# ratschlab/projects2014-metagenome

Hardware: AMD Instinct MI355X
Metric: k-mers/s ingested into BOSS (k=31, 150 bp reads) (higher is better)
Workload: dtype u64

## Files before the change

projects2014-metagenome_amd/csrc/boss_pipeline.hip:

```cpp
#include <hip/hip_runtime.h>

#include <algorithm>
#include <cmath>
#include <atomic>
#include <chrono>
#include <cstdio>
#include <cstring>
#include <mutex>
#include <stdexcept>
#include <string>
#include <type_traits>
#include <vector>

#include <sys/types.h>
#include <unistd.h>

#include "../../include/mtg_boss.h"
#include "boss_kernels.hpp"
#include "comm.hpp"
#include "dbg_io.hpp"
#include "dbg_device.hpp"
#include "dist_kernels.hpp"
#include "superkmer.hpp"
#include "extract_partition.hpp"
// ... 658 lines not shown
template <int L>
static MsdPlan msd_plan(const Ctx &c, uint64_t n, unsigned nbits, double dup) {
    const double LIMIT = (double)LocalTraits<L>::LIMIT / 2;
    const unsigned dmax = MSD_DBITS;
    unsigned T = 0;
    while (T < nbits && T < 3 * dmax && (double)n / dup / (double)(1ull << T) > LIMIT / kPlanDiv)
        ++T;
    MsdPlan p{};
    p.levels = (T + dmax - 1) / dmax;
    if (c.min_levels > p.levels && T >= c.min_levels) p.levels = c.min_levels;
    for (unsigned l = 1; l <= p.levels; ++l) p.digit_end[l] = T * l / p.levels;
    return p;
}

static void note_bucket_index(Ctx &c, const void *keys, uint64_t n, const uint64_t *start, unsigned shift);

template <int L>
static MsdPlan rc_plan(const Ctx &c, uint64_t n, unsigned nbits) {
    return msd_plan<L>(c, L == 2 && c.rc_wide ? std::max<uint64_t>(1, n / 2) : n, nbits, 1.0);
}

template <int L>
struct RcMerge {
    const Key<L> *ck;
    const uint32_t *cv;
    uint64_t nc;
    Key<L> *out;
    uint32_t *outc;
    bool done = false;
    uint64_t *istart = nullptr;
    unsigned ib = 0;
};

__global__ void spec_caps_kernel(const uint32_t *__restrict__ sample, uint64_t nb, uint32_t stride,
                                 uint32_t *__restrict__ cap, bool tiny, uint64_t blo, uint64_t bhi,
                                 uint32_t align = 0) {
    const uint64_t b = (uint64_t)blockIdx.x * blockDim.x + threadIdx.x;
    if (b >= nb) return;
    if (b < blo || b >= bhi) {
        cap[b] = 0;
        return;
    }
    uint32_t v = tiny ? (uint32_t)(((uint64_t)sample[b] * stride) / 2)
                      : (uint32_t)(((uint64_t)sample[b] * stride * 6) / 5) + 512u;
    if (align) v = (v + align - 1) / align * align;
    cap[b] = v;
}

__global__ void spec_tile_fill_kernel(const uint64_t *__restrict__ bstart, const unsigned long long *__restrict__ cur,
                                      uint64_t nb, uint32_t tile, uint32_t *__restrict__ tv) {
    const uint64_t b = (uint64_t)blockIdx.x * blockDim.x + threadIdx.x;
    if (b >= nb) return;
    const uint64_t s = bstart[b], e = bstart[b + 1], k = cur[b];
    for (uint64_t t = s / tile; t < e / tile; ++t) {
        const uint64_t t0 = t * tile;
        tv[t] = (uint32_t)(k <= t0 ? 0 : min<uint64_t>(tile, k - t0));
    }
}

__global__ void spec_counts_kernel(const uint64_t *__restrict__ bstart, const unsigned long long *__restrict__ cur,
                                   uint64_t nb, uint32_t *__restrict__ cnt) {
    const uint64_t b = (uint64_t)blockIdx.x * blockDim.x + threadIdx.x;
    if (b < nb) cnt[b] = (uint32_t)(cur[b] - bstart[b]);
}

template <typename F>
static void bucket_pieces(uint64_t lo, uint64_t hi, F &&launch) {
    constexpr uint64_t CH = 1ull << 22;
    for (uint64_t g0 = lo; g0 < hi; g0 += CH) launch(g0, (unsigned)std::min(CH, hi - g0));
}

static void ensure_compact(Ctx &c) {
    if (!c.gap.valid) return;
    c.gap.valid = false;
    if (!c.gap.nb) return;
    bucket_pieces(0, c.gap.nb, [&](uint64_t g0, unsigned cnt) {
        group_gather_kernel<1, false><<<dim3(cnt), dim3(256), 0, c.stream>>>(
            (const Key<1> *)c.gap.keys, nullptr, c.gap.bstart, c.gap.ustart, (Key<1> *)c.gap.dst, nullptr, nullptr, 0,
            nullptr, nullptr, g0);
        HIP_CHECK(hipGetLastError());
    });
}

template <int L, bool COUNTED>
static uint64_t spec_final_level(Ctx &c, Key<L> **keys, uint32_t **vals, uint64_t n, unsigned nbits, unsigned bp,
                                 unsigned bb, uint32_t cmax, bool distinct, RcMerge<L> *rm,
                                 const Ctx::GroupIndex &cidx, bool fine = false, Key<L> *spare = nullptr) {
    if constexpr (L != 1) {
        return ~0ull;
    } else {
        constexpr double KB = COUNTED ? 12.0 : 8.0;
        if (distinct != (rm != nullptr)) return ~0ull;
        if (rm && !c.spec_rc) return ~0ull;
        if (rm && !(cidx.keys == (const void *)rm->ck && cidx.n == rm->nc && cidx.bits == bb && cidx.nbits == nbits &&
                    bb <= 32 && (!rm->istart || rm->ib >= bb)))
            return ~0ull;
        constexpr uint32_t SS = 8;
        constexpr int TILE = MsdTraits<L>::TILE;
        const bool g1 = bp && c.gap1_n && !rm;
        const uint64_t npos = g1 ? c.gap1_n : n;
        const uint32_t *tv = g1 ? c.gap1_tv : nullptr;
        const uint64_t tiles = ceil_div(npos, TILE);
        if (c.use_lsd || !c.spec_final || tiles < 64 * SS || bb - bp > 9 || bb > 24) return ~0ull;
        if (g1) fine = true;
        const uint64_t nb = 1ull << bb;
        const bool gap_out = !COUNTED && c.defer_gather_req && c.defer_gather && c.want_gidx;
        const bool inplace = !rm && c.spec_inplace && !gap_out;
        if (COUNTED) spare = nullptr;
        if (!spare) {
            const uint64_t fr = c.ws.free_bytes();
            if ((double)n * KB * 1.4 * (inplace ? 1.0 : 2.0) > 0.5 * (double)fr + (double)c.ws.held_slot(Workspace::SPEC_A) +
                                                  (double)c.ws.held_slot(Workspace::SPEC_B) +
                                                  (double)c.ws.held_slot(Workspace::SPEC_AC) +
                                                  (double)c.ws.held_slot(Workspace::SPEC_BC))
                return ~0ull;
        }
        uint32_t *h = (uint32_t *)c.ws.get(Workspace::MSD_COUNTS, nb * 4);
        HIP_CHECK(hipMemsetAsync(h, 0, nb * 4, c.stream));
        constexpr uint32_t GT = 8;
        msd_hist_kernel<L><<<dim3((unsigned)(fine ? ceil_div(tiles, GT) : ceil_div(tiles, SS))), dim3(MSD_BLOCK), 0,
                             c.stream>>>(*keys, npos, nbits, bb, bp, h, fine ? 1 : SS, fine ? SS : 1, fine ? GT : 1, tv);
        HIP_CHECK(hipGetLastError());
        uint64_t blo = 0, bhi = nb;
        if (g1 && c.gap1_hi > c.gap1_lo) {
            blo = c.gap1_lo << (bb - bp);
            bhi = std::min<uint64_t>(nb, c.gap1_hi << (bb - bp));
        } else if (bp && !g1) {
            Key<L> ends[2];
            HIP_CHECK(hipMemcpyAsync(&ends[0], *keys, sizeof(Key<L>), hipMemcpyDeviceToHost, c.stream));
            HIP_CHECK(hipMemcpyAsync(&ends[1], *keys + (n - 1), sizeof(Key<L>), hipMemcpyDeviceToHost, c.stream));
            HIP_CHECK(hipStreamSynchronize(c.stream));
            blo = (ends[0].w[0] >> (nbits - bp)) << (bb - bp);
            bhi = std::min<uint64_t>(nb, ((ends[1].w[0] >> (nbits - bp)) + 1) << (bb - bp));
        }
        uint32_t *cap = (uint32_t *)c.ws.get(Workspace::SPEC_CAP, nb * 4);
        spec_caps_kernel<<<dim3((unsigned)ceil_div(nb, 256)), dim3(256), 0, c.stream>>>(h, nb, SS, cap, c.spec_tiny,
                                                                                        blo, bhi);
        HIP_CHECK(hipGetLastError());
        uint64_t *bstart = (uint64_t *)c.ws.get(Workspace::MSD_BSTART, (nb + 1) * 8);
        {
            uint32_t ep;
            const uint64_t st = ceil_div(nb, 4096);
            uint64_t *desc = acquire_desc(c, st, &ep);
            HIP_CHECK(hipMemsetAsync(&c.small->counter, 0, 4, c.stream));
            scan_counts_kernel<<<dim3((unsigned)st), dim3(512), 0, c.stream>>>(cap, nb, bstart, desc, ep,
                                                                              &c.small->counter, &c.small->error);
            HIP_CHECK(hipGetLastError());
        }
        const uint64_t C = read_u64(c, (const unsigned long long *)(bstart + nb));
        if (spare && C * sizeof(Key<L>) > c.spec_into_bytes) spare = nullptr;
        if (!spare) {
            const uint64_t fr = c.ws.free_bytes();
            const double need = (double)C * KB * (rm || inplace ? 1.0 : 2.0);
            const double have = 0.9 * (double)fr + (double)c.ws.held_slot(Workspace::SPEC_A) +
                                (double)c.ws.held_slot(Workspace::SPEC_AC) +
                                (rm ? 0.0 : (double)c.ws.held_slot(Workspace::SPEC_B) +
                                                (double)c.ws.held_slot(Workspace::SPEC_BC));
            if (need > have) {
                if (c.debug) fprintf(stderr, "[mtg debug] speculative level: capacity %lu does not fit, exact level\n",
                                     (unsigned long)C);
                return ~0ull;
            }
        }
        Key<L> *sa = spare ? spare : (Key<L> *)c.ws.get(Workspace::SPEC_A, C * sizeof(Key<L>));
        uint32_t *sac = COUNTED ? (uint32_t *)c.ws.get(Workspace::SPEC_AC, C * 4) : nullptr;
        auto *cur = (unsigned long long *)c.ws.get(Workspace::SPEC_CUR, nb * 8);
        HIP_CHECK(hipMemcpyAsync(cur, bstart, nb * 8, hipMemcpyDeviceToDevice, c.stream));
        HIP_CHECK(hipMemsetAsync(&c.small->spec_ovf, 0, 4, c.stream));
        EventTimer tm(c.stream);
        tm.mark();
        msd_partition_kernel<L, COUNTED><<<dim3((unsigned)xcd_grid(tiles)), dim3(MSD_BLOCK), 0, c.stream>>>(
            *keys, sa, COUNTED ? *vals : nullptr, sac, npos, nbits, bb, bp, cur, 1,
            (const unsigned long long *)(bstart + 1), &c.small->spec_ovf, tv);
        HIP_CHECK(hipGetLastError());
        tm.mark();
        uint32_t povf = 0;
        HIP_CHECK(hipMemcpyAsync(&povf, &c.small->spec_ovf, 4, hipMemcpyDeviceToHost, c.stream));
        HIP_CHECK(hipStreamSynchronize(c.stream));
        if (c.track_partition && c.radix_launches == 0) {
            c.radix_ms += tm.ms(0, 1);
            c.radix_launches += 1;
            c.radix_bytes += 2.0 * n * KB;
        }
        if (povf) {
            if (c.debug) fprintf(stderr, "[mtg debug] speculative level: a bucket overflowed, exact level\n");
            c.radix_ms = 0, c.radix_launches = 0, c.radix_bytes = 0;
            ++c.timings.spec_fallbacks;
            return ~0ull;
        }
        auto consumed_gap1 = [&]() {
            if (g1) c.gap1_n = 0, c.gap1_tv = nullptr, c.gap1_lo = c.gap1_hi = 0;
        };
        if (rm) {
            uint32_t *cnt = (uint32_t *)c.ws.get(Workspace::SPEC_CAP, nb * 4);
            spec_counts_kernel<<<dim3((unsigned)ceil_div(nb, 256)), dim3(256), 0, c.stream>>>(bstart, cur, nb, cnt);
            HIP_CHECK(hipGetLastError());
            uint64_t *gbase = (uint64_t *)c.ws.get(Workspace::MSD_USTART, (nb + 1) * 8);
            {
                uint32_t ep;
                const uint64_t st = ceil_div(nb, 4096);
                uint64_t *desc = acquire_desc(c, st, &ep);
                HIP_CHECK(hipMemsetAsync(&c.small->counter, 0, 4, c.stream));
                scan_counts_kernel<<<dim3((unsigned)st), dim3(512), 0, c.stream>>>(cnt, nb, gbase, desc, ep,
                                                                                  &c.small->counter, &c.small->error);
                HIP_CHECK(hipGetLastError());
            }
            constexpr int CAP = MergeLocalTraits<L>::CAP;
            uint32_t *olist = (uint32_t *)c.ws.get(Workspace::MSD_OVF, nb * 4);
            HIP_CHECK(hipMemsetAsync(&c.small->counter, 0, 4, c.stream));
            uint64_t *istart = rm->istart;
            const bool gapped = c.gap.valid && c.gap.dst == (const void *)rm->ck;
            const Key<L> *ck = gapped ? (const Key<L> *)c.gap.keys : rm->ck;
            const uint64_t *cgap = gapped ? c.gap.bstart : nullptr;
            uint64_t mlo = 0, mhi = nb;
            if (bp && !g1 && !gapped && rm->nc) {
                Key<L> e[4];
                HIP_CHECK(hipMemcpyAsync(&e[0], *keys, sizeof(Key<L>), hipMemcpyDeviceToHost, c.stream));
                HIP_CHECK(hipMemcpyAsync(&e[1], *keys + (n - 1), sizeof(Key<L>), hipMemcpyDeviceToHost, c.stream));
                HIP_CHECK(hipMemcpyAsync(&e[2], rm->ck, sizeof(Key<L>), hipMemcpyDeviceToHost, c.stream));
                HIP_CHECK(hipMemcpyAsync(&e[3], rm->ck + (rm->nc - 1), sizeof(Key<L>), hipMemcpyDeviceToHost, c.stream));
                HIP_CHECK(hipStreamSynchronize(c.stream));
                auto top = [&](const Key<L> &x) { return bits_at(shr(x, nbits - bp), 0, 32); };
                mlo = std::min(top(e[0]), top(e[2])) << (bb - bp);
                mhi = std::min<uint64_t>(nb, (std::max(top(e[1]), top(e[3])) + 1) << (bb - bp));
                if (istart && mlo < mhi) {
                    const uint64_t ilo = mlo << (rm->ib - bb), ihi = mhi << (rm->ib - bb), iend = 1ull << rm->ib;
                    if (ilo) fill_u64_kernel<<<dim3((unsigned)std::min<uint64_t>(ceil_div(ilo, 256), 4096)), dim3(256), 0,
                                               c.stream>>>(istart, 0, ilo, 0);
                    if (ihi < iend)
                        fill_u64_kernel<<<dim3((unsigned)std::min<uint64_t>(ceil_div(iend - ihi, 256), 4096)), dim3(256),
                                          0, c.stream>>>(istart, ihi, iend, n + rm->nc);
                    HIP_CHECK(hipGetLastError());
                } else if (mlo >= mhi) {
                    mlo = 0, mhi = nb;
                }
            }
            bucket_pieces(mlo, mhi, [&](uint64_t g0, unsigned cnt) {
                local_merge_kernel<L, COUNTED, CAP><<<dim3(cnt), dim3(512), 0, c.stream>>>(
                    sa, sac, bstart, nullptr, nullptr, ck, rm->cv, cidx.start, rm->out, rm->outc, olist,
                    &c.small->counter, bb, nbits, rm->ib, istart, cur, gbase, cgap, g0, c.merge_it);
                HIP_CHECK(hipGetLastError());
            });
            uint32_t novf = 0;
            HIP_CHECK(hipMemcpyAsync(&novf, &c.small->counter, 4, hipMemcpyDeviceToHost, c.stream));
            HIP_CHECK(hipStreamSynchronize(c.stream));
            if (novf) {
                const uint32_t nlist = novf;
                HIP_CHECK(hipMemsetAsync(&c.small->counter, 0, 4, c.stream));
                bucket_pieces(0, nlist, [&](uint64_t g0, unsigned cnt) {
                    local_merge_kernel<L, COUNTED, 2 * CAP><<<dim3(cnt), dim3(512), 0, c.stream>>>(
                        sa, sac, bstart, nullptr, olist + g0, ck, rm->cv, cidx.start, rm->out, rm->outc, nullptr,
                        &c.small->counter, bb, nbits, rm->ib, istart, cur, gbase, cgap, 0, c.merge_it);
                    HIP_CHECK(hipGetLastError());
                });
                HIP_CHECK(hipMemcpyAsync(&novf, &c.small->counter, 4, hipMemcpyDeviceToHost, c.stream));
                HIP_CHECK(hipStreamSynchronize(c.stream));
// ... 79 lines not shown
                fprintf(stderr, "[mtg debug] speculative level: n=%lu capacity=%lu (%.2fx) -> %lu distinct, left in buckets\n",
                        (unsigned long)n, (unsigned long)C, (double)C / (double)n, (unsigned long)u);
            return u;
        }
        const bool index = c.want_gidx;
        const bool rindex = !index && c.ridx.start && bb <= c.ridx.bits;
        uint64_t *gi = index ? (uint64_t *)c.ws.get(Workspace::CANON_IDX, (nb + 2) * 8) : rindex ? c.ridx.start : nullptr;
        const unsigned ib = rindex ? c.ridx.bits : bb;
        if (index || rindex) HIP_CHECK(hipMemsetAsync(&c.small->gidx_bad, 0, 4, c.stream));
        if (c.sort_out && (c.sort_out_cap == ~0ull || read_u64(c, (const unsigned long long *)(ustart + nb)) <= c.sort_out_cap)) {
            *keys = (Key<L> *)c.sort_out;
            if (COUNTED) *vals = c.sort_out_vals;
        }
        bucket_pieces(0, nb, [&](uint64_t g0, unsigned cnt) {
            group_gather_kernel<L, COUNTED><<<dim3(cnt), dim3(256), 0, c.stream>>>(
                sb, sbc, bstart, ustart, *keys, COUNTED ? *vals : nullptr, nullptr, nbits - ib, gi, &c.small->gidx_bad,
                g0, ib - bb, rindex ? c.ridx.off : 0, rindex ? c.ridx.lo : 0, rindex ? c.ridx.hi : ~0ull);
            HIP_CHECK(hipGetLastError());
        });
        uint64_t u = 0;
        uint32_t ibad = 0;
        HIP_CHECK(hipMemcpyAsync(&u, ustart + nb, 8, hipMemcpyDeviceToHost, c.stream));
        if (index) {
            HIP_CHECK(hipMemcpyAsync(gi + nb, ustart + nb, 8, hipMemcpyDeviceToDevice, c.stream));
            HIP_CHECK(hipMemcpyAsync(gi + nb + 1, ustart + nb, 8, hipMemcpyDeviceToDevice, c.stream));
        }
        if (index || rindex) HIP_CHECK(hipMemcpyAsync(&ibad, &c.small->gidx_bad, 4, hipMemcpyDeviceToHost, c.stream));
        HIP_CHECK(hipStreamSynchronize(c.stream));
        if (index && !ibad) c.gidx = Ctx::GroupIndex{*keys, u, bb, nbits, gi};
        if (rindex) c.ridx.written = !ibad;
        consumed_gap1();
        ++c.timings.spec_levels;
        if (fine) ++c.timings.spec_fine_levels;
        if (c.debug)
            fprintf(stderr, "[mtg debug] speculative level: n=%lu capacity=%lu (%.2fx) -> %lu distinct\n",
                    (unsigned long)n, (unsigned long)C, (double)C / (double)n, (unsigned long)u);
        return u;
    }
}

template <int L, bool COUNTED>
static bool spec_mid_level(Ctx &c, Key<L> **keys, Key<L> **alt, uint64_t n, unsigned nbits, unsigned bp, unsigned bb) {
    if constexpr (L != 1 || COUNTED) {
        return false;
    } else {
        constexpr int TILE = MsdTraits<L>::TILE;
        constexpr uint32_t SS = 8;
        const uint64_t tiles = ceil_div(n, TILE);
        if (c.use_lsd || !c.spec_final || tiles < 64 * SS || bb - bp > 9 || bb > 24 || !bp) return false;
        const uint64_t nb = 1ull << bb;
        uint32_t *h = (uint32_t *)c.ws.get(Workspace::MSD_COUNTS, nb * 4);
        HIP_CHECK(hipMemsetAsync(h, 0, nb * 4, c.stream));
        msd_hist_kernel<L><<<dim3((unsigned)ceil_div(tiles, SS)), dim3(MSD_BLOCK), 0, c.stream>>>(*keys, n, nbits, bb, bp, h,
                                                                                                SS, 1, 1, nullptr);
        HIP_CHECK(hipGetLastError());
        Key<L> ends[2];
        HIP_CHECK(hipMemcpyAsync(&ends[0], *keys, sizeof(Key<L>), hipMemcpyDeviceToHost, c.stream));
        HIP_CHECK(hipMemcpyAsync(&ends[1], *keys + (n - 1), sizeof(Key<L>), hipMemcpyDeviceToHost, c.stream));
        HIP_CHECK(hipStreamSynchronize(c.stream));
        const uint64_t lo1 = ends[0].w[0] >> (nbits - bp), hi1 = ends[1].w[0] >> (nbits - bp);
        const uint64_t blo = lo1 << (bb - bp), bhi = std::min<uint64_t>(nb, (hi1 + 1) << (bb - bp));
        uint32_t *cap = (uint32_t *)c.ws.get(Workspace::SPEC_CAP, nb * 4);
        spec_caps_kernel<<<dim3((unsigned)ceil_div(nb, 256)), dim3(256), 0, c.stream>>>(h, nb, SS, cap, c.spec_tiny, blo,
                                                                                        bhi, (uint32_t)TILE);
        HIP_CHECK(hipGetLastError());
        uint64_t *bstart = (uint64_t *)c.ws.get(Workspace::MSD_BSTART, (nb + 1) * 8);
        {
            uint32_t ep;
            const uint64_t st = ceil_div(nb, 4096);
            uint64_t *desc = acquire_desc(c, st, &ep);
            HIP_CHECK(hipMemsetAsync(&c.small->counter, 0, 4, c.stream));
            scan_counts_kernel<<<dim3((unsigned)st), dim3(512), 0, c.stream>>>(cap, nb, bstart, desc, ep,
                                                                              &c.small->counter, &c.small->error);
            HIP_CHECK(hipGetLastError());
        }
        const uint64_t C = read_u64(c, (const unsigned long long *)(bstart + nb));
        if (C * sizeof(Key<L>) > c.spec_mid_bytes) {
            if (c.debug) fprintf(stderr, "[mtg debug] speculative middle level: capacity %lu does not fit\n", (unsigned long)C);
            return false;
        }
        auto *cur = (unsigned long long *)c.ws.get(Workspace::SPEC_CUR, nb * 8);
        HIP_CHECK(hipMemcpyAsync(cur, bstart, nb * 8, hipMemcpyDeviceToDevice, c.stream));
        HIP_CHECK(hipMemsetAsync(&c.small->spec_ovf, 0, 4, c.stream));
        msd_partition_kernel<L, false><<<dim3((unsigned)xcd_grid(tiles)), dim3(MSD_BLOCK), 0, c.stream>>>(
            *keys, *alt, nullptr, nullptr, n, nbits, bb, bp, cur, 1, (const unsigned long long *)(bstart + 1),
            &c.small->spec_ovf, nullptr);
        HIP_CHECK(hipGetLastError());
        const uint64_t ntv = C / TILE;
        uint32_t *tv = (uint32_t *)c.ws.get(Workspace::SPEC_MID_TV, std::max<uint64_t>(ntv, 1) * 4);
        spec_tile_fill_kernel<<<dim3((unsigned)ceil_div(nb, 256)), dim3(256), 0, c.stream>>>(bstart, cur, nb, TILE, tv);
        HIP_CHECK(hipGetLastError());
        uint32_t povf = 0;
        HIP_CHECK(hipMemcpyAsync(&povf, &c.small->spec_ovf, 4, hipMemcpyDeviceToHost, c.stream));
        HIP_CHECK(hipStreamSynchronize(c.stream));
        if (povf) {
            if (c.debug) fprintf(stderr, "[mtg debug] speculative middle level: a bucket overflowed, exact level\n");
            ++c.timings.spec_fallbacks;
            return false;
        }
        std::swap(*keys, *alt);
        c.gap1_n = C;
        c.gap1_tv = tv;
        c.gap1_lo = blo, c.gap1_hi = bhi;
        ++c.timings.spec_levels;
        if (c.debug)
            fprintf(stderr, "[mtg debug] speculative middle level: n=%lu capacity=%lu (%.2fx)\n", (unsigned long)n,
                    (unsigned long)C, (double)C / (double)n);
        return true;
    }
}

template <int L, bool COUNTED>
static uint64_t msd_sort_unique(Ctx &c, Key<L> **keys, Key<L> **alt, uint32_t **vals,
                                uint32_t **valt, uint64_t n, unsigned nbits, uint32_t cmax,
                                double dup, const uint32_t *hist1 = nullptr, bool distinct = false,
                                const std::vector<uint64_t> *runs = nullptr, bool level1_done = false,
                                RcMerge<L> *rm = nullptr, const MsdPlan *force_plan = nullptr) {
    const Ctx::GroupIndex saved_gidx = c.gidx;
    c.gidx = Ctx::GroupIndex{};
    if (n == 0) return 0;
    auto lazy_alt = [&]() {
        if (!*alt) *alt = (Key<L> *)c.ws.get(Workspace::KB, n * sizeof(Key<L>));
        if (COUNTED && !*valt) *valt = (uint32_t *)c.ws.get(Workspace::CB, n * 4);
    };
    constexpr uint32_t LIMIT = LocalTraits<L>::LIMIT;
    constexpr int TILE = MsdTraits<L>::TILE;
    const uint64_t tiles = ceil_div(n, TILE);
    const MsdPlan plan = force_plan ? *force_plan : msd_plan<L>(c, n, nbits, dup);
    unsigned levels = plan.levels;
    unsigned digit_end[4] = {plan.digit_end[0], plan.digit_end[1], plan.digit_end[2], plan.digit_end[3]};
    unsigned b = 0;
    uint64_t *bstart = nullptr;
    uint64_t nbuckets = 1;
    auto run_level = [&](unsigned lev) {
        if (digit_end[lev] == 0) digit_end[lev] = std::min(nbits, digit_end[lev - 1] + 8);
        const unsigned bb = digit_end[lev], bp = digit_end[lev - 1];
        nbuckets = 1ull << bb;
        const uint32_t *cnt = hist1;
        const bool g1 = c.gap1_n && (lev == 2 ? level1_done : lev == 3);
        const uint64_t npos = g1 ? c.gap1_n : n, ltiles = g1 ? ceil_div(npos, TILE) : tiles;
        const uint32_t *tv = g1 ? c.gap1_tv : nullptr;
        if (lev != 1 || !hist1) {
            uint32_t *h = (uint32_t *)c.ws.get(Workspace::MSD_COUNTS, nbuckets * 4);
            HIP_CHECK(hipMemsetAsync(h, 0, nbuckets * 4, c.stream));
            if (bp == 0 && nbuckets <= 512) {
                const uint32_t nrows = (uint32_t)std::min<uint64_t>(tiles, 8192);
                uint32_t *rows = (uint32_t *)c.ws.get(Workspace::HIST_ROWS, (uint64_t)nrows * nbuckets * 4);
                msd_hist_rows_kernel<L><<<dim3(nrows), dim3(512), 0, c.stream>>>(*keys, n, nbits, bb, rows);
                HIP_CHECK(hipGetLastError());
                hist_rows_reduce_kernel<<<dim3(std::min<uint32_t>(nrows, 256), (unsigned)ceil_div(nbuckets, 256)),
                                          dim3(256), 0, c.stream>>>(rows, nrows, (uint32_t)nbuckets, h);
            } else {
                msd_hist_kernel<L><<<dim3((unsigned)ltiles), dim3(MSD_BLOCK), 0, c.stream>>>(*keys, npos, nbits, bb, bp,
                                                                                             h, 1, 1, 1, tv);
            }
            HIP_CHECK(hipGetLastError());
            cnt = h;
        }
        bstart = (uint64_t *)c.ws.get(Workspace::MSD_BSTART, (nbuckets + 1) * 8);
        uint32_t ep;
        const uint64_t st = ceil_div(nbuckets, 4096);
        uint64_t *desc = acquire_desc(c, st, &ep);
        HIP_CHECK(hipMemsetAsync(&c.small->counter, 0, 4, c.stream));
        scan_counts_kernel<<<dim3((unsigned)st), dim3(512), 0, c.stream>>>(cnt, nbuckets, bstart, desc, ep,
                                                                      &c.small->counter, &c.small->error);
        HIP_CHECK(hipGetLastError());
        if (lev == 1 && level1_done) {
            b = bb;
            return;
        }
        lazy_alt();
        auto *cur = (unsigned long long *)c.ws.get(Workspace::MSD_CURSOR, nbuckets * 8);
        HIP_CHECK(hipMemcpyAsync(cur, bstart, nbuckets * 8, hipMemcpyDeviceToDevice, c.stream));
        EventTimer tm(c.stream);
        tm.mark();
        msd_partition_kernel<L, COUNTED><<<dim3((unsigned)xcd_grid(ltiles)), dim3(MSD_BLOCK), 0, c.stream>>>(
            *keys, *alt, COUNTED ? *vals : nullptr, COUNTED ? *valt : nullptr, npos, nbits, bb, bp, cur, 1, nullptr,
            nullptr, tv);
        HIP_CHECK(hipGetLastError());
        if (g1) c.gap1_n = 0, c.gap1_tv = nullptr, c.gap1_lo = c.gap1_hi = 0;
        tm.mark();
        if (c.track_partition && c.radix_launches == 0) {
            HIP_CHECK(hipStreamSynchronize(c.stream));
            c.radix_ms += tm.ms(0, 1);
            c.radix_launches += 1;
            c.radix_bytes += 2.0 * n * (sizeof(Key<L>) + (COUNTED ? 4 : 0));
        }
        std::swap(*keys, *alt);
        if (COUNTED) std::swap(*vals, *valt);
        b = bb;
    };
    if (runs && runs->size() >= 2 && runs->size() <= 129 && levels) {
        lazy_alt();
        const unsigned T = digit_end[levels];
        const uint32_t P = (uint32_t)runs->size() - 1;
        nbuckets = 1ull << T;
        uint64_t *idx = (uint64_t *)c.ws.get(Workspace::RUN_IDX, (uint64_t)P * (nbuckets + 1) * 8);
        int64_t *delta = (int64_t *)c.ws.get(Workspace::RUN_DELTA, (uint64_t)P * nbuckets * 8);
        for (uint32_t j = 0; j < P; ++j) {
            const uint64_t r0 = (*runs)[j], rn = (*runs)[j + 1] - r0;
            bucket_index<L>(c, *keys + r0, rn, nbits - T, nbuckets, idx + (uint64_t)j * (nbuckets + 1));
        }
        bstart = (uint64_t *)c.ws.get(Workspace::MSD_BSTART, (nbuckets + 1) * 8);
        runs_delta_kernel<<<dim3((unsigned)std::min<uint64_t>(ceil_div(nbuckets + 1, 256), 16384)), dim3(256), 0,
                            c.stream>>>(idx, P, nbuckets, bstart, delta);
        HIP_CHECK(hipGetLastError());
        uint64_t *droff = (uint64_t *)c.ws.get(Workspace::RUN_OFF, (P + 1) * 8);
        HIP_CHECK(hipMemcpyAsync(droff, runs->data(), (P + 1) * 8, hipMemcpyHostToDevice, c.stream));
        runs_gather_kernel<L, COUNTED><<<dim3((unsigned)std::min<uint64_t>(ceil_div(n, 256), 65536)), dim3(256), 0,
                                         c.stream>>>(*keys, COUNTED ? *vals : nullptr, n, droff, P, delta,
                                                     nbuckets, nbits, T, *alt, COUNTED ? *valt : nullptr);
        HIP_CHECK(hipGetLastError());
        HIP_CHECK(hipStreamSynchronize(c.stream));
        std::swap(*keys, *alt);
        if (COUNTED) std::swap(*vals, *valt);
        b = T;
    } else {
        for (unsigned lev = 1; lev <= levels; ++lev) {
            if (lev == levels && lev >= 2 && (lev == 2 || c.spec3) && (level1_done || (rm && distinct) || (!rm && !distinct))) {
                const bool fine = lev >= 3 || (n >> digit_end[lev - 1]) < 64ull * MsdTraits<L>::TILE;
                Key<L> *spare = lev >= 3 && c.spec_into && c.spec_into != (void *)*keys ? (Key<L> *)c.spec_into : nullptr;
                const uint64_t u = spec_final_level<L, COUNTED>(c, keys, vals, n, nbits, digit_end[lev - 1],
                                                                digit_end[lev], cmax, distinct, rm, saved_gidx, fine,
                                                                spare);
                if (u != ~0ull) return u;
            }
            if (lev == 2 && levels == 3 && level1_done && !c.gap1_n && c.spec_mid && c.spec3 && *alt &&
                c.spec_mid_into == (void *)*alt &&
                spec_mid_level<L, COUNTED>(c, keys, alt, n, nbits, digit_end[1], digit_end[2])) {
                b = digit_end[2];
                continue;
            }
            run_level(lev);
        }
    }

    lazy_alt();
    while (true) {
        const uint64_t G = LIMIT / 4;
        uint64_t ngroups = 1;
        uint64_t *gstart;
        const uint64_t *gbucket_out = nullptr;
        if (b == 0) {
            gstart = (uint64_t *)c.ws.get(Workspace::MSD_GSTART, 16);
            set_pair_kernel<<<1, 1, 0, c.stream>>>(gstart, 0, n);
            HIP_CHECK(hipGetLastError());
        } else {
            uint32_t *gf = (uint32_t *)c.ws.get(Workspace::MSD_UCOUNT, (nbuckets + 1) * 4);
            const bool fuse = rm && distinct && b <= 32;
            uint64_t *cstart = nullptr;
            const uint64_t *gsize = bstart;
            if (fuse) {
                ensure_compact(c);
                if (saved_gidx.keys == (const void *)rm->ck && saved_gidx.n == rm->nc && saved_gidx.bits == b &&
                    saved_gidx.nbits == nbits) {
                    cstart = const_cast<uint64_t *>(saved_gidx.start);
                } else {
                    cstart = (uint64_t *)c.ws.get(Workspace::RC_CSTART, (nbuckets + 2) * 8);
                    bucket_index<L>(c, rm->ck, rm->nc, nbits - b, nbuckets, cstart);
                }
                uint64_t *comb = (uint64_t *)c.ws.get(Workspace::RC_COMB, (nbuckets + 1) * 8);
// ... 5127 lines not shown
```

projects2014-metagenome_amd/csrc/msd_sort.hpp:

```cpp
#pragma once

#include "device_common.hpp"
#include "keys.hpp"

namespace mtg {


constexpr int MSD_BLOCK = 512;
constexpr int MSD_WIN = 2;
constexpr int MSD_DBITS = 9;

template <int L>
struct MsdTraits {
    static constexpr int ITEMS = L == 1 ? 16 : L == 2 ? 8 : 4;
    static constexpr int TILE = ITEMS * MSD_BLOCK;
};

template <int L>
__device__ __forceinline__ uint32_t key_prefix(const Key<L> &k, unsigned nbits, unsigned bits) {
    return bits ? bits_at(k, nbits - bits, bits) : 0u;
}

template <int L>
__global__ __launch_bounds__(MSD_BLOCK) void msd_hist_kernel(const Key<L> *__restrict__ keys,
// ... 76 lines not shown
    __shared__ uint32_t s_h[512];
    const uint32_t nb = 1u << b;
    for (uint32_t i = threadIdx.x; i < nb; i += 512) s_h[i] = 0;
    __syncthreads();
    const uint64_t stride = (uint64_t)gridDim.x * 512;
    if constexpr (L == 1) {
        for (uint64_t p = (uint64_t)blockIdx.x * 512 + threadIdx.x; 2 * p < n; p += stride) {
            const uint64_t i = 2 * p;
            if (i + 1 < n) {
                const ulonglong2 v = *(const ulonglong2 *)(keys + i);
                atomicAdd(&s_h[key_prefix(Key<L>::from(v.x), nbits, b)], 1u);
                atomicAdd(&s_h[key_prefix(Key<L>::from(v.y), nbits, b)], 1u);
            } else {
                atomicAdd(&s_h[key_prefix(keys[i], nbits, b)], 1u);
            }
        }
    } else {
        for (uint64_t i = (uint64_t)blockIdx.x * 512 + threadIdx.x; i < n; i += stride)
            atomicAdd(&s_h[key_prefix(keys[i], nbits, b)], 1u);
    }
    __syncthreads();
    for (uint32_t i = threadIdx.x; i < nb; i += 512) rows[(uint64_t)blockIdx.x * nb + i] = s_h[i];
}

__global__ __launch_bounds__(256) void hist_rows_reduce_kernel(const uint32_t *__restrict__ rows,
                                                               uint32_t nrows, uint32_t nb,
                                                               uint32_t *__restrict__ out) {
    const uint32_t bin = blockIdx.y * 256 + threadIdx.x;
    if (bin >= nb) return;
    uint32_t sum = 0;
    for (uint32_t r = blockIdx.x; r < nrows; r += gridDim.x) sum += rows[(uint64_t)r * nb + bin];
    if (sum) atomicAdd(&out[bin], sum);
}

__global__ __launch_bounds__(512) void scan_counts_kernel(const uint32_t *__restrict__ counts,
                                                          uint64_t n, uint64_t *__restrict__ starts,
                                                          uint64_t *desc, uint32_t epoch,
                                                          uint32_t *tile_counter, uint32_t *error) {
    constexpr int ITEMS = 8, TILE = 512 * ITEMS;
    __shared__ uint64_t s_scan[512 / 64 + 1];
    __shared__ uint32_t s_tile;
    __shared__ uint64_t s_base;
    const uint32_t tile = take_tile(tile_counter, &s_tile);
    const uint64_t i0 = (uint64_t)tile * TILE + (uint64_t)threadIdx.x * ITEMS;
    uint32_t v[ITEMS];
    uint64_t sum = 0;
#pragma unroll
    for (int j = 0; j < ITEMS; ++j) {
        v[j] = i0 + j < n ? counts[i0 + j] : 0;
        sum += v[j];
    }
    uint64_t tile_total;
    const uint64_t off = block_exclusive_sum_u64<512>(sum, s_scan, &tile_total);
    tile_base_lookback(desc, tile, tile_total, epoch, error, &s_base);
    uint64_t s = s_base + off;
#pragma unroll
    for (int j = 0; j < ITEMS; ++j) {
        if (i0 + j < n) starts[i0 + j] = s;
        s += v[j];
    }
    const uint64_t ntiles = (n + TILE - 1) / TILE;
    if (tile + 1 == ntiles && threadIdx.x == 511) starts[n] = s_base + tile_total;
}

template <int L>
__device__ __forceinline__ Key<L> load_key(const Key<L> *p, bool nt) {
    if (!nt) return *p;
    Key<L> k;
#pragma unroll
    for (int i = 0; i < L; ++i) k.w[i] = __builtin_nontemporal_load(&p->w[i]);
    return k;
}

template <int L>
__device__ __forceinline__ void store_key(Key<L> *p, const Key<L> &k, bool nt) {
    if (nt) {
#pragma unroll
        for (int i = 0; i < L; ++i) __builtin_nontemporal_store(k.w[i], &p->w[i]);
    } else {
        *p = k;
    }
}

template <int L, bool HAS_VAL, int BLOCK = MSD_BLOCK, bool NT = false>
__global__ __launch_bounds__(BLOCK) void msd_partition_kernel(
    const Key<L> *__restrict__ kin, Key<L> *__restrict__ kout, const uint32_t *__restrict__ vin,
    uint32_t *__restrict__ vout, uint64_t n, unsigned nbits, unsigned b, unsigned bp,
    unsigned long long *__restrict__ cursor, unsigned cstride = 1,
    const unsigned long long *__restrict__ bend = nullptr, uint32_t *__restrict__ povf = nullptr,
    const uint32_t *__restrict__ tvalid = nullptr) {
    constexpr int ITEMS = MsdTraits<L>::ITEMS;
    constexpr int TILE = ITEMS * BLOCK;
    constexpr int WMAX = MSD_WIN << 8;
    __shared__ Key<L> s_keys[TILE];
    __shared__ uint32_t s_vals[HAS_VAL ? TILE : 1];
    __shared__ uint32_t s_cnt[WMAX];
    __shared__ uint32_t s_loff[WMAX];
    __shared__ unsigned long long s_gbase[WMAX];
    __shared__ uint32_t s_scan[BLOCK / 64 + 1];

    const uint32_t tid = threadIdx.x;
    const uint64_t tile = xcd_tile((n + TILE - 1) / TILE);
    if (tile * TILE >= n) return;
    const uint32_t tv = tvalid ? tvalid[tile] : (uint32_t)TILE;
    if (tv == 0) return;
    const uint64_t base = tile * TILE;
    const unsigned sub = b - bp;
    const uint32_t wsize = min((uint32_t)WMAX, (uint32_t)MSD_WIN << sub);
    for (int i = tid; i < (int)wsize; i += BLOCK) s_cnt[i] = 0;
    const uint32_t wbase = key_prefix(kin[base], nbits, bp) << sub;
    __syncthreads();

    Key<L> k[ITEMS];
    uint32_t v[ITEMS];
    uint32_t r[ITEMS];
    bool have[ITEMS];
#pragma unroll
    for (int j = 0; j < ITEMS; ++j) {
        const uint64_t i = base + (uint64_t)j * BLOCK + tid;
        have[j] = i < n && (uint32_t)j * BLOCK + tid < tv;
        if (have[j]) {
            k[j] = load_key(kin + i, NT);
            if (HAS_VAL) v[j] = vin[i];
        }
    }
#pragma unroll
    for (int j = 0; j < ITEMS; ++j) {
        r[j] = 0xFFFFFFFFu;
        if (have[j]) {
            const uint32_t lb = key_prefix(k[j], nbits, b) - wbase;
            if (lb < wsize) {
                r[j] = atomicAdd(&s_cnt[lb], 1u);
            } else {
                const unsigned long long o = atomicAdd(&cursor[(size_t)(lb + wbase) * cstride], 1ull);
                if (bend && o >= bend[lb + wbase]) {
                    *povf = 1u;
                } else {
                    kout[o] = k[j];
                    if (HAS_VAL) vout[o] = v[j];
                }
            }
        }
    }
    __syncthreads();
    constexpr int PER = WMAX / BLOCK > 0 ? WMAX / BLOCK : 1;
    uint32_t c[PER];
    uint32_t sum = 0;
#pragma unroll
    for (int q = 0; q < PER; ++q) {
        const uint32_t i = tid * PER + q;
        c[q] = i < wsize ? s_cnt[i] : 0;
        sum += c[q];
    }
    uint32_t total;
    uint32_t off = block_exclusive_sum<BLOCK>(sum, s_scan, &total);
    unsigned long long gq[PER], be[PER];
#pragma unroll
    for (int q = 0; q < PER; ++q) {
        const uint32_t i = tid * PER + q;
        gq[q] = 0, be[q] = 0;
        if (i < wsize) {
            s_loff[i] = off;
            if (c[q]) {
                gq[q] = atomicAdd(&cursor[(size_t)(wbase + i) * cstride], (unsigned long long)c[q]);
                if (bend) be[q] = bend[wbase + i];
            }
        }
        off += c[q];
    }
    __syncthreads();
#pragma unroll
    for (int j = 0; j < ITEMS; ++j) {
        if (r[j] != 0xFFFFFFFFu) {
            const uint32_t lb = key_prefix(k[j], nbits, b) - wbase;
            const uint32_t pos = s_loff[lb] + r[j];
            s_keys[pos] = k[j];
            if (HAS_VAL) s_vals[pos] = v[j];
        }
    }
#pragma unroll
    for (int q = 0; q < PER; ++q) {
        const uint32_t i = tid * PER + q;
        if (i < wsize) {
            unsigned long long gb = gq[q];
            if (bend && c[q] && gb + c[q] > be[q]) {
                *povf = 1u;
                gb = ~0ull;
            }
            s_gbase[i] = gb;
        }
    }
    __syncthreads();
    for (uint32_t p = tid; p < total; p += BLOCK) {
        const Key<L> key = s_keys[p];
        const uint32_t lb = key_prefix(key, nbits, b) - wbase;
        if (bend && s_gbase[lb] == ~0ull) continue;
        const uint64_t o = s_gbase[lb] + (p - s_loff[lb]);
        store_key(kout + o, key, NT);
        if (HAS_VAL) vout[o] = s_vals[p];
    }
}

__global__ void group_flags_kernel(const uint64_t *__restrict__ bstart, uint64_t nbuckets,
                                   uint64_t G, uint32_t *__restrict__ flags) {
    const uint64_t b = (uint64_t)blockIdx.x * blockDim.x + threadIdx.x;
    if (b >= nbuckets) return;
    const uint64_t s0 = bstart[b], s1 = bstart[b + 1];
    uint32_t f = 0;
    if (s1 > s0) {
        if (b == 0 || s0 == 0) {
            f = 1;
        } else {
            uint64_t p = b;
            uint64_t ps = s0;
            while (p > 0 && bstart[p - 1] == s0) --p;
            if (p > 0) ps = bstart[p - 1];
            f = (s0 / G != ps / G) || (s1 - s0 > G) || (s0 - ps > G);
        }
    }
    flags[b] = f;
}

__global__ void add_starts_kernel(const uint64_t *__restrict__ a, const uint64_t *__restrict__ b, uint64_t n,
                                  uint64_t *__restrict__ c) {
    const uint64_t i = (uint64_t)blockIdx.x * blockDim.x + threadIdx.x;
    if (i < n) c[i] = a[i] + b[i];
}

__global__ void group_scatter_kernel(const uint64_t *__restrict__ bstart,
                                     const uint32_t *__restrict__ flags,
                                     const uint64_t *__restrict__ pos, uint64_t nbuckets,
                                     uint64_t n, uint64_t *__restrict__ gstart,
                                     uint64_t *__restrict__ gbucket = nullptr) {
    const uint64_t b = (uint64_t)blockIdx.x * blockDim.x + threadIdx.x;
    if (b < nbuckets && flags[b]) {
        gstart[pos[b]] = bstart[b];
        if (gbucket) gbucket[pos[b]] = pos[b] == 0 ? 0 : b;
    }
    if (b == nbuckets) {
        gstart[pos[nbuckets]] = n;
        if (gbucket) gbucket[pos[nbuckets]] = nbuckets;
    }
}

__global__ void runs_delta_kernel(const uint64_t *__restrict__ idx, uint32_t P, uint64_t nb,
                                  uint64_t *__restrict__ bstart, int64_t *__restrict__ delta) {
    const uint64_t stride = (uint64_t)gridDim.x * blockDim.x;
    for (uint64_t b = (uint64_t)blockIdx.x * blockDim.x + threadIdx.x; b <= nb; b += stride) {
        uint64_t s = 0;
        for (uint32_t j = 0; j < P; ++j) s += idx[(uint64_t)j * (nb + 1) + b];
        bstart[b] = s;
        if (b == nb) continue;
        uint64_t o = s;
        for (uint32_t j = 0; j < P; ++j) {
            const uint64_t lo = idx[(uint64_t)j * (nb + 1) + b], hi = idx[(uint64_t)j * (nb + 1) + b + 1];
            delta[(uint64_t)j * nb + b] = (int64_t)o - (int64_t)lo;
            o += hi - lo;
        }
    }
}

template <int L, bool HAS_VAL>
__global__ __launch_bounds__(256) void runs_gather_kernel(const Key<L> *__restrict__ kin,
                                                          const uint32_t *__restrict__ vin, uint64_t n,
                                                          const uint64_t *__restrict__ roff, uint32_t P,
                                                          const int64_t *__restrict__ delta, uint64_t nb,
                                                          unsigned nbits, unsigned T, Key<L> *__restrict__ kout,
                                                          uint32_t *__restrict__ vout) {
    __shared__ uint64_t s_off[129];
    for (uint32_t j = threadIdx.x; j <= P; j += blockDim.x) s_off[j] = roff[j];
    __syncthreads();
    const uint64_t stride = (uint64_t)gridDim.x * blockDim.x;
    for (uint64_t i = (uint64_t)blockIdx.x * blockDim.x + threadIdx.x; i < n; i += stride) {
        uint32_t j = 0;
        while (j + 1 < P && s_off[j + 1] <= i) ++j;
        const Key<L> k = kin[i];
        const uint32_t b = key_prefix(k, nbits, T);
        const uint64_t o = (uint64_t)((int64_t)(i - s_off[j]) + delta[(uint64_t)j * nb + b]);
        kout[o] = k;
        if (HAS_VAL) vout[o] = vin[i];
// ... 682 lines not shown
```

Before: 55.47 billion.

## Run uncounted u64 MSD partition with 1024-thread blocks and per-bucket deltas

For single-word keys without counts, the MSD partition kernel now launches with 1024-thread blocks and 8 items per thread, keeping the same tile size, and requests 8 waves per EU. The scatter phase stores one precomputed delta per bucket (global base minus local offset) in shared memory, so each element needs one LDS lookup instead of two, and a sentinel marks refused runs. The larger block changes the scan, the atomic count per thread and register pressure, and may reduce occupancy if the waves-per-EU hint cannot be met.

```diff
diff --git a/projects2014-metagenome_amd/csrc/boss_pipeline.hip b/projects2014-metagenome_amd/csrc/boss_pipeline.hip
--- a/projects2014-metagenome_amd/csrc/boss_pipeline.hip
+++ b/projects2014-metagenome_amd/csrc/boss_pipeline.hip
@@ -764,6 +764,16 @@
     });
 }
 
+template <int L, bool COUNTED, typename... A>
+static void launch_msd_partition(Ctx &c, uint64_t tiles, A... a) {
+    if constexpr (L == 1 && !COUNTED) {
+        static_assert(MsdTraits<1>::TILE == 8 * 1024, "the same tile");
+        msd_partition_kernel<1, false, 1024, false, 8><<<dim3((unsigned)xcd_grid(tiles)), dim3(1024), 0, c.stream>>>(a...);
+    } else {
+        msd_partition_kernel<L, COUNTED><<<dim3((unsigned)xcd_grid(tiles)), dim3(MSD_BLOCK), 0, c.stream>>>(a...);
+    }
+}
+
 template <int L, bool COUNTED>
 static uint64_t spec_final_level(Ctx &c, Key<L> **keys, uint32_t **vals, uint64_t n, unsigned nbits, unsigned bp,
                                  unsigned bb, uint32_t cmax, bool distinct, RcMerge<L> *rm,
@@ -851,9 +861,8 @@
         HIP_CHECK(hipMemsetAsync(&c.small->spec_ovf, 0, 4, c.stream));
         EventTimer tm(c.stream);
         tm.mark();
-        msd_partition_kernel<L, COUNTED><<<dim3((unsigned)xcd_grid(tiles)), dim3(MSD_BLOCK), 0, c.stream>>>(
-            *keys, sa, COUNTED ? *vals : nullptr, sac, npos, nbits, bb, bp, cur, 1,
-            (const unsigned long long *)(bstart + 1), &c.small->spec_ovf, tv);
+        launch_msd_partition<L, COUNTED>(c, tiles, *keys, sa, COUNTED ? *vals : nullptr, sac, npos, nbits, bb, bp, cur, 1,
+                                         (const unsigned long long *)(bstart + 1), &c.small->spec_ovf, tv);
         HIP_CHECK(hipGetLastError());
         tm.mark();
         uint32_t povf = 0;
@@ -1099,9 +1108,8 @@
         auto *cur = (unsigned long long *)c.ws.get(Workspace::SPEC_CUR, nb * 8);
         HIP_CHECK(hipMemcpyAsync(cur, bstart, nb * 8, hipMemcpyDeviceToDevice, c.stream));
         HIP_CHECK(hipMemsetAsync(&c.small->spec_ovf, 0, 4, c.stream));
-        msd_partition_kernel<L, false><<<dim3((unsigned)xcd_grid(tiles)), dim3(MSD_BLOCK), 0, c.stream>>>(
-            *keys, *alt, nullptr, nullptr, n, nbits, bb, bp, cur, 1, (const unsigned long long *)(bstart + 1),
-            &c.small->spec_ovf, nullptr);
+        launch_msd_partition<L, false>(c, tiles, *keys, *alt, nullptr, nullptr, n, nbits, bb, bp, cur, 1,
+                                       (const unsigned long long *)(bstart + 1), &c.small->spec_ovf, nullptr);
         HIP_CHECK(hipGetLastError());
         const uint64_t ntv = C / TILE;
         uint32_t *tv = (uint32_t *)c.ws.get(Workspace::SPEC_MID_TV, std::max<uint64_t>(ntv, 1) * 4);
@@ -1191,9 +1199,8 @@
         HIP_CHECK(hipMemcpyAsync(cur, bstart, nbuckets * 8, hipMemcpyDeviceToDevice, c.stream));
         EventTimer tm(c.stream);
         tm.mark();
-        msd_partition_kernel<L, COUNTED><<<dim3((unsigned)xcd_grid(ltiles)), dim3(MSD_BLOCK), 0, c.stream>>>(
-            *keys, *alt, COUNTED ? *vals : nullptr, COUNTED ? *valt : nullptr, npos, nbits, bb, bp, cur, 1, nullptr,
-            nullptr, tv);
+        launch_msd_partition<L, COUNTED>(c, ltiles, *keys, *alt, COUNTED ? *vals : nullptr, COUNTED ? *valt : nullptr, npos,
+                                         nbits, bb, bp, cur, 1, nullptr, nullptr, tv);
         HIP_CHECK(hipGetLastError());
         if (g1) c.gap1_n = 0, c.gap1_tv = nullptr, c.gap1_lo = c.gap1_hi = 0;
         tm.mark();
diff --git a/projects2014-metagenome_amd/csrc/msd_sort.hpp b/projects2014-metagenome_amd/csrc/msd_sort.hpp
--- a/projects2014-metagenome_amd/csrc/msd_sort.hpp
+++ b/projects2014-metagenome_amd/csrc/msd_sort.hpp
@@ -182,21 +182,24 @@
     }
 }
 
-template <int L, bool HAS_VAL, int BLOCK = MSD_BLOCK, bool NT = false>
-__global__ __launch_bounds__(BLOCK) void msd_partition_kernel(
+constexpr unsigned long long RUN_REFUSED = 1ull << 63;
+
+template <int L, bool HAS_VAL, int BLOCK = MSD_BLOCK, bool NT = false, int ITEMS_ = MsdTraits<L>::ITEMS>
+__global__ __launch_bounds__(BLOCK) __attribute__((amdgpu_waves_per_eu(BLOCK == 1024 && ITEMS_ <= 8 ? 8 : 1)))
+void msd_partition_kernel(
     const Key<L> *__restrict__ kin, Key<L> *__restrict__ kout, const uint32_t *__restrict__ vin,
     uint32_t *__restrict__ vout, uint64_t n, unsigned nbits, unsigned b, unsigned bp,
     unsigned long long *__restrict__ cursor, unsigned cstride = 1,
     const unsigned long long *__restrict__ bend = nullptr, uint32_t *__restrict__ povf = nullptr,
     const uint32_t *__restrict__ tvalid = nullptr) {
-    constexpr int ITEMS = MsdTraits<L>::ITEMS;
+    constexpr int ITEMS = ITEMS_;
     constexpr int TILE = ITEMS * BLOCK;
     constexpr int WMAX = MSD_WIN << 8;
     __shared__ Key<L> s_keys[TILE];
     __shared__ uint32_t s_vals[HAS_VAL ? TILE : 1];
     __shared__ uint32_t s_cnt[WMAX];
     __shared__ uint32_t s_loff[WMAX];
-    __shared__ unsigned long long s_gbase[WMAX];
+    __shared__ unsigned long long s_delta[WMAX];
     __shared__ uint32_t s_scan[BLOCK / 64 + 1];
 
     const uint32_t tid = threadIdx.x;
@@ -255,10 +258,12 @@
     uint32_t total;
     uint32_t off = block_exclusive_sum<BLOCK>(sum, s_scan, &total);
     unsigned long long gq[PER], be[PER];
+    uint32_t lo[PER];
 #pragma unroll
     for (int q = 0; q < PER; ++q) {
         const uint32_t i = tid * PER + q;
         gq[q] = 0, be[q] = 0;
+        lo[q] = off;
         if (i < wsize) {
             s_loff[i] = off;
             if (c[q]) {
@@ -285,17 +290,18 @@
             unsigned long long gb = gq[q];
             if (bend && c[q] && gb + c[q] > be[q]) {
                 *povf = 1u;
-                gb = ~0ull;
-            }
-            s_gbase[i] = gb;
+                s_delta[i] = RUN_REFUSED;
+            } else {
+                s_delta[i] = gb - lo[q];
+            }
         }
     }
     __syncthreads();
     for (uint32_t p = tid; p < total; p += BLOCK) {
         const Key<L> key = s_keys[p];
-        const uint32_t lb = key_prefix(key, nbits, b) - wbase;
-        if (bend && s_gbase[lb] == ~0ull) continue;
-        const uint64_t o = s_gbase[lb] + (p - s_loff[lb]);
+        const unsigned long long d = s_delta[key_prefix(key, nbits, b) - wbase];
+        if (d == RUN_REFUSED) continue;
+        const uint64_t o = p + d;
         store_key(kout + o, key, NT);
         if (HAS_VAL) vout[o] = s_vals[p];
     }
```

New measurement: 55.98 billion, median of 6. Within noise of the previous version (+0.9%).
